# feinanshan/TDNet

Hardware: AMD Instinct MI355X
Metric: frames/sec (td4-psp18, 1024x2048, full-resolution logits) (higher is better)
Workload: dtype f32; 1 GPU; td4-psp18, 1024x2048 Cityscapes-shaped synthetic stream, 3-frame feature cache, 1 clip per GPU; parallelism=clip-parallel x1, RCCL weight broadcast only, target_fps_per_gpu=30

## Files before the change

tdnet_amd/csrc/td_launch.h:

```cpp
#pragma once
#include "td_weights.h"

#ifdef TDNET_TIMING_PROBES
static int probe_skip() {
    static const int m = [] {
        const char* e = getenv("TDNET_PROBE_SKIP");
        const int v = e ? atoi(e) : 0;
        if (v) fprintf(stderr, "tdnet: TDNET_PROBE_SKIP=%d -- pieces of the frame are NOT computed, every result of this process is garbage (timing probe build)\n", v);
        return v;
    }();
    return m;
}
#else
static constexpr int probe_skip() { return 0; }
#endif
static void prof_begin(tdnet* n, int family, int dominant, double flops, hipStream_t s) {
    if (!n || !n->prof) return;
    if (n->nrec == n->recs.size()) {
        ProfRec r;
        hipEventCreate(&r.e0); hipEventCreate(&r.e1);
        n->recs.push_back(r);
    }
    ProfRec& r = n->recs[n->nrec];
    r.family = family; r.dominant = dominant; r.flops = flops;
// ... 44 lines not shown
    const int TY = wino_tiles_1d(H, L.dil, L.wino), TX = wino_tiles_1d(W, L.dil, L.wino);
    const long T = (long)L.dil * L.dil * TY * TX;
    const bool chunked = ck.ny != 1 || ck.nx != 1;
    if (chunked && (!L.vw || L.dil % ck.ny || L.dil % ck.nx)) return td_fail("internal: this conv cannot run in chunks");
    const long Tc = (long)(L.dil / ck.ny) * (L.dil / ck.nx) * TY * TX;
    const int nb = (L.wino + 2) * (L.wino + 2);
    bool own = false;
    if (!V) {
        own = n == nullptr || n->wino_v_floats < (size_t)nb * Tc * L.Cin || n->wino_m_floats < (size_t)nb * Tc * L.Cout;
        if (own) {
            if (n) { n->failed = true; return td_fail("internal: Winograd workspace too small"); }
            if (dev_alloc(&V, (size_t)nb * Tc * L.Cin) || dev_alloc(&Mb, (size_t)nb * Tc * L.Cout)) return -1;
        } else { V = n->wino_v; Mb = n->wino_m; }
    }
    WinoArgs wa;
    wa.in = in; wa.V = V; wa.Mb = Mb; wa.bias = L.d_bias; wa.resid = resid; wa.out = out;
    wa.H = H; wa.W = W; wa.C = L.Cin; wa.Cout = L.Cout; wa.dil = L.dil; wa.TY = TY; wa.TX = TX; wa.T = (int)T; wa.act = L.act; wa.TP = (int)Tc;
    wa.ln_mean = lnf ? lnf->mean : nullptr; wa.ln_rstd = lnf ? lnf->rstd : nullptr; wa.ln_g = lnf ? lnf->g : nullptr; wa.ln_b = lnf ? lnf->b : nullptr;
    wa.Tc = (int)Tc; wa.ny = ck.ny; wa.cy = ck.cy; wa.nx = ck.nx; wa.cx = ck.cx;
    const long cmax = L.Cin > L.Cout ? L.Cin : L.Cout;
    if ((long)nb * Tc * cmax * 4 >= (1l << 31) || (long)H * W * cmax * 4 >= (1l << 31) ||
        (L.vw && !(wino_magic_ok(Tc * ((cmax + 63) / 64), TX) && wino_magic_ok(0, TY) && wino_magic_ok(0, L.dil))))
        return td_fail("internal: this conv is too large for the Winograd transforms");
    wa.mg_sl = wino_magic(1); wa.mg_tx = wino_magic(TX); wa.mg_ty = wino_magic(TY); wa.pw = L.dil / ck.nx; wa.mg_pw = wino_magic(wa.pw);
    auto transform = [&](bool out_side) {
        if (n && (probe_skip() & 1)) return;
        prof_begin(n, 2, false, 0, s);
        const int C = out_side ? L.Cout : L.Cin;
        if (out_side && cls) {
            const unsigned grid = (unsigned)((Tc + 3) / 4);
            if (L.Cout == 128) TD_LAUNCH((k_wino4_out_cls<2>), dim3(grid), dim3(256), wino_out_cls_lds(128, cls->NC), s, wa, *cls);
            else TD_LAUNCH((k_wino4_out_cls<1>), dim3(grid), dim3(256), wino_out_cls_lds(64, cls->NC), s, wa, *cls);
        } else
        if (L.vw == 1) launch_wino4_c<1>(out_side, wa, s);
        else if (L.vw == 2 && C % 2 == 0) launch_wino4_c<2>(out_side, wa, s);
        else if (L.vw == 4 && C % 4 == 0) launch_wino4_c<4>(out_side, wa, s);
        else if (L.vw) launch_wino4_c<1>(out_side, wa, s);
        else if (out_side && wino_act_general(wa.act)) TD_LAUNCH((k_wino4_out<true>), dim3(td_grid_for(T * (L.Cout / 4), 256, 256 * 16)), dim3(256), 0, s, wa);
        else if (out_side) TD_LAUNCH((k_wino4_out<false>), dim3(td_grid_for(T * (L.Cout / 4), 256, 256 * 16)), dim3(256), 0, s, wa);
        else TD_LAUNCH(k_wino4_in, dim3(td_grid_for(T * (L.Cin / 4), 256, 256 * 16)), dim3(256), 0, s, wa);
        prof_end(n, s);
    };
    transform(false);
    prof_begin(n, 0, 2, 2.0 * nb * Tc * (double)L.Cin * L.Cout, s);
    if (!(n && (probe_skip() & 8))) launch_gemm(L, gemm_args(L, V, (int)Tc, nb, L.d_zero, nullptr, Mb, 0), chunked ? 320 : 0, s);
    prof_end(n, s);
    transform(true);
    if (own) { TD_HIP(hipStreamSynchronize(s)); hipFree(V); hipFree(Mb); }
    return 0;
}

static void launch_conv_dma_forms(const ConvLayer& L, const ConvArgs& a, hipStream_t s) {
    int rh = L.rh;
    bool done = false;
    const bool is192 = rh == CD_192_P || rh == CD_192_N;
    if (rh == CD_128_N || rh == CD_192_N) {
        done = !L.rowimg_off && conv_launch_dma3n(a, rh, L.KS, L.out16, s);
        if (!done) rh = is192 ? CD_192_P : CD_128_P;
    }
    if (!done && (rh == CD_128_P || rh == CD_192_P)) {
        done = !L.rowimg_off && conv_launch_dma3p(a, rh, L.KS, L.out16, s);
        if (!done) rh = is192 ? CD_192 : CD_128_8W;
    }
    if (!done && (L.rowimg_off || !conv_launch_dma3(a, rh, L.KS, L.out16, s))) conv_launch_dma(a, rh, L.KS, L.out16, s);
}

static int run_conv(tdnet* n, const ConvLayer& L, const float* in, int H, int W, const float* resid, float* out, hipStream_t s,
                    int* Ho_out = nullptr, int* Wo_out = nullptr, const LnFuse* lnf = nullptr, const ClsArgs* cls = nullptr) {
    if (lnf && !L.wino) return td_fail("internal: LayerNorm fusion needs a Winograd input transform");
    if (cls && (!L.wino || L.chunks > 1 || resid || wino_act_general(L.act))) return td_fail("internal: the classifier rides in a whole Winograd conv's output transform");
    const int Ho = out_size(H, L.KS, L.stride, L.dil, L.pad), Wo = out_size(W, L.KS, L.stride, L.dil, L.pad);
    if (L.wino) {
        if (Ho_out) *Ho_out = H;
        if (Wo_out) *Wo_out = W;
        if (L.chunks > 1 && (!n || !n->ws_ready)) {
            for (int c = 0; c < L.chunks; ++c) {
                WinoChunk ck; ck.ny = L.chunks; ck.cy = c;
                TD_TRY(run_wino(n, L, in, H, W, resid, out, s, lnf, ck, nullptr, nullptr));
            }
            return 0;
        }
        return run_wino(n, L, in, H, W, resid, out, s, lnf, WinoChunk(), nullptr, nullptr, cls);
    }
    if (L.route == CR_WINO_F64 && !wino_f64_size_ok(H, W)) return td_fail("internal: this map is too large for the fused Winograd kernel");
    const ConvArgs a = conv_args(L, in, H, W, resid, out);
    const double flops = L.route == CR_WINO_F64 ? 2.0 * 36 * (double)wino_tiles(H, W, 1, 4) * L.Cin * L.Cout : L.flops_per_pixel() * a.M;
    prof_begin(n, 0, (((L.tile == CT_128x128 || L.tile == CT_128x128_DEEP || L.rh) && L.KS == 3 && !L.stem) ? 1 : 0) | ((L.h16() && L.in16 && L.KS == 3 && !L.stem) ? 4 : 0), flops, s);
    switch (L.route) {
    case CR_STEM_H: conv_launch_stem_h(a, L.out16, s); break;
    case CR_CONV_DMA: launch_conv_dma_forms(L, a, s); break;
    case CR_CONV_H: conv_launch_h(a, L.tile, L.KS, L.in16, L.out16, s); break;
    case CR_ADIRECT_B3: conv_launch_adirect_b3(a, L.KS, 0, s); break;
    case CR_GEMM1X1: launch_gemm(L, gemm_args(L, in, a.M, 1, L.d_bias, resid, out, L.act), 0, s); break;
    case CR_ADIRECT_ROWS:
    case CR_ADIRECT_ROWS_B3: {
        ConvArgs r = a;
        r.H = stem_rows_hp(H); r.W = stem_rows_wp(W); r.Cin = 3; r.pad = 0;
        if (L.route == CR_ADIRECT_ROWS_B3) conv_launch_adirect_b3(r, L.KS, 2, s);
        else conv_launch_adirect(r, L.KS, 2, s);
        break;
    }
    case CR_ADIRECT: conv_launch_adirect(a, L.KS, L.stem ? 1 : 0, s); break;
    case CR_IGEMM: conv_launch(a, L.tile, L.KS, L.stem, s); break;
    case CR_WINO_F64: wino_f64_launch(in, L.d_wp, L.d_bias, resid, out, H, W, L.act, s); break;
    case CR_WINO: break;
    }
    prof_end(n, s);
    if (Ho_out) *Ho_out = Ho;
    if (Wo_out) *Wo_out = Wo;
    return 0;
}

static int run_conv_src2(tdnet* n, const ConvLayer& L, const float* in, int ld, int k_split, int nsteps, const float* in2, int ld2, const float* wp2,
                         int H, int W, const float* resid, float* out, hipStream_t s) {
    if (L.KS != 1 || L.stem || L.wino) return td_fail("internal: two operand sources need a 1x1 conv");
    const ConvArgs a0 = conv_args(L, in, H, W, resid, out);
    prof_begin(n, 0, 0, 2.0 * L.Cout * 32.0 * nsteps * a0.M, s);
    int rc = 0;
    if (L.route == CR_GEMM1X1 && L.gemm == GK_PERSISTENT) {
        GemmArgs ga = gemm_args(L, in, a0.M, 1, L.d_bias, resid, out, L.act);
        ga.K = 32 * nsteps; ga.k_split = k_split; ga.lda = ld; ga.a2 = in2; ga.lda2 = ld2; ga.wp2 = wp2;
        if (!gemm_src2_supports(ga)) rc = td_fail("internal: the persistent GEMM cannot take this second operand source");
        else launch_gemm(L, ga, 0, s);
    } else if (L.route == CR_ADIRECT) {
        ConvArgs a = a0;
        a.Cin = 32 * nsteps; a.nsteps = nsteps; a.k_split = k_split; a.ld = ld; a.in2 = in2; a.ld2 = ld2; a.wp2 = wp2;
        if (resid || !conv_adirect_src2_supports(a, L.KS, 0)) rc = td_fail("internal: the direct 1x1 conv cannot take this second operand source");
        else conv_launch_adirect(a, 1, 0, s);
    } else rc = td_fail("internal: this conv's kernel has no second operand source");
    prof_end(n, s);
    return rc;
}

struct ConvCall { const ConvLayer* L; const float* in; int H, W; float* out; };
static bool conv_group_same_form(const tdnet_opts& o, const ConvCall* c, int ng) {
    bool same = (o.fusion & TDNET_FUSION_CONV_GROUPS) && ng >= 2 && ng <= 3;
    for (int g = 0; same && g < ng; ++g) {
        const ConvLayer& L = *c[g].L;
        const ConvLayer& L0 = *c[0].L;
        same = L.route == CR_CONV_H && L.in16 == L.out16 && L.in16 == L0.in16 && (g == 0 ? (L.KS == 1 || L.KS == 3) : L.KS == 1) &&
               conv_tile_dims(L.tile).BM == conv_tile_dims(L0.tile).BM && conv_tile_dims(L.tile).BN == conv_tile_dims(L0.tile).BN;
    }
    return same;
}
static int run_conv_group(tdnet* n, const tdnet_opts& o, const ConvCall* c, int ng, hipStream_t s, int* Ho_out = nullptr, int* Wo_out = nullptr,
                          int* grouped = nullptr) {
    const bool same = conv_group_same_form(o, c, ng);
    if (grouped) *grouped = same ? 1 : 0;
    if (!same) {
        for (int g = 0; g < ng; ++g) TD_TRY(run_conv(n, *c[g].L, c[g].in, c[g].H, c[g].W, nullptr, c[g].out, s, g == 0 ? Ho_out : nullptr, g == 0 ? Wo_out : nullptr));
        return 0;
    }
    ConvArgs a[3];
    double flops = 0.0;
    for (int g = 0; g < ng; ++g) {
        const ConvLayer& L = *c[g].L;
        a[g] = conv_args(L, c[g].in, c[g].H, c[g].W, nullptr, c[g].out);
        flops += L.flops_per_pixel() * a[g].M;
        if (g == 0 && Ho_out) *Ho_out = out_size(c[0].H, L.KS, L.stride, L.dil, L.pad);
        if (g == 0 && Wo_out) *Wo_out = a[0].Wo;
    }
    const bool dom = c[0].L->in16 && c[0].L->KS == 3;
    prof_begin(n, 0, dom ? 4 : 0, dom ? c[0].L->flops_per_pixel() * a[0].M : flops, s);
    conv_launch_h_group(a, ng, c[0].L->tile, c[0].L->KS, c[0].L->in16, c[0].L->out16, s);
    prof_end(n, s);
    return 0;
}

static int run_attention(tdnet* n, const float* q, const float* k, const float* vp, const float* bias, const float* resid,
                         int Lq, int Lk, int DV, float* out, hipStream_t s, int online = 0, float* ln_part = nullptr,
                         _Float16* vt16 = nullptr, bool slices = false, bool vt_ready = false, int b3 = 0) {
    if (n && n->vt16 && (n->opts.precision == 1 || b3)) vt16 = n->vt16;
    AttnArgs a;
    a.q = q; a.k = k; a.vp = vp; a.bias = bias; a.resid = resid; a.out = out; a.Lq = Lq; a.Lk = Lk;
    a.scale_log2e = 1.4426950408889634f / 8.0f;
    a.ln_part = ln_part; a.ln_nstr = 0;
    if (n && (probe_skip() & 4) && Lq > Lk) return 0;
    prof_begin(n, 1, false, 2.0 * Lq * (double)Lk * (64 + DV), s);
    const int rc = (vt16 && b3) ? attn_launch_b3(a, DV, reinterpret_cast<unsigned short*>(vt16), s, vt_ready, b3 - 1)
                 : vt16 ? attn_launch_h(a, DV, vt16, s, vt_ready) : attn_launch(a, DV, online, s, slices);
    prof_end(n, s);
    if (rc) return td_fail("attention: unsupported d_v=%d (128 or a multiple of 512)", DV);
    return 0;
}

static void run_layernorm(tdnet* n, const float* x, int HW, int C, const float* g, const float* b, float* part, float* mean,
                          float* rstd, float* y, hipStream_t s, int stats_nstr = 0, bool y16 = false) {
// ... 399 lines not shown
```

tdnet_amd/csrc/td_weights.h:

```cpp
#pragma once
#include "td_handle.h"

constexpr int RH_FRAME = -1;
constexpr int RH_BY_SIZE = -2;

static int plan_dma_form(const ConvLayer& c, long M, const tdnet_opts& o) {
    const bool narrow = (o.fusion & TDNET_FUSION_DMA_NARROW) != 0, same3 = c.KS == 3 && c.stride == 1 && c.pad == c.dil;
    if (!conv_dma_supports(c.Cin, c.Cout, c.KS, c.tile)) return CD_NONE;
    if (c.Cout == 64 && c.CoutPad == 128 && same3 && narrow) return CD_128_N;
    if (c.Cout < 128) return CD_NONE;
    const int rh = conv_dma_pick_rh(M, c.Cout, c.CoutPad % 256 == 0);
    if (narrow && same3 && M <= 16384 && c.Cout <= 256) return c.Cout <= 128 ? CD_128_N : CD_192_N;
    if (o.fusion & TDNET_FUSION_DMA_LOADERS) return rh == CD_128 ? CD_128_P : rh == CD_192 ? CD_192_P : rh;
    return rh;
}

static bool plan_wino_f64(const tdnet_opts& o, int Cout, int Cin, int KS, int stride, int dil, int act, bool stem, bool forced_tile, int chunks) {
    return (o.fusion & TDNET_FUSION_WINO_F64) && o.winograd >= 3 && o.precision == 0 && !forced_tile && chunks == 1 &&
           wino_f64_supports(Cout, Cin, KS, stride, dil, act, stem);
}

static int plan_conv(ConvLayer& L, int Cout, int Cin, int KS, int stride, int dil, int act, bool stem, long M, const tdnet_opts& o,
                     int forced_tile = -1, int chunks = 1, bool in16 = false, bool out16 = false, int rh = RH_FRAME, bool rowimg_off = false) {
    L = ConvLayer();
    L.Cin = stem ? 4 : Cin; L.Cout = Cout; L.KS = KS; L.stride = stride; L.dil = dil; L.act = act; L.stem = stem;
    L.pad = stem ? KS / 2 : dil * (KS / 2);
    L.pers = o.gemm_persistent;
    L.rowimg_off = rowimg_off;
    if (!stem && Cin % 32 != 0) return td_fail("conv: Cin=%d is not a multiple of 32", Cin);
    const bool deep = o.pipeline != 0, forced = forced_tile >= 0;
    const bool pers_gemm = o.gemm_persistent && gemm_supports(Cin);
    const bool split = o.precision >= 2;
    const bool split_narrow = split && (o.fusion & TDNET_FUSION_A_DIRECT) && (o.fusion & TDNET_FUSION_SPLIT_NARROW);
    if (plan_wino_f64(o, Cout, Cin, KS, stride, dil, act, stem, forced, chunks) && M >= TD_WINO_F64_MIN_PIXELS && M <= TD_WINO_F64_MAX_PIXELS) {
        L.route = CR_WINO_F64;
        L.nsteps = 0; L.CoutPad = Cout;
        return 0;
    }
    if (o.winograd && o.precision != 1 && !stem && KS == 3 && stride == 1 && Cin % 32 == 0 && Cout % 4 == 0 && (o.winograd == 4 || (Cin >= 128 && Cout >= 128))) {
        L.route = CR_WINO;
        L.wino = 4;
        L.chunks = (chunks > 1 && dil % chunks == 0 && pers_gemm) ? chunks : 1;
        L.vw = (L.chunks > 1 || (o.overlap & TDNET_OVERLAP_LOWREG_TRANSFORMS)) ? (1 << ((o.overlap & TDNET_OVERLAP_VW_MASK) >> TDNET_OVERLAP_VW_SHIFT)) : 0;
        const int nb = (L.wino + 2) * (L.wino + 2);
        const long rows = wino_tiles_estimate(M, dil, L.wino) / L.chunks;
        L.tile = forced ? (ConvTile)forced_tile : pers_gemm ? gemm_pick_tile(rows, nb, Cout, deep)
                                                            : conv_pick_tile((int)std::min<long>(nb * M / (L.wino * L.wino), 1 << 30), Cout, deep);
        L.nsteps = conv_nsteps(Cin, 1, 0);
        const bool b3 = split && pers_gemm && gemm_b3_supports(Cin, Cout) && (forced || o.precision == 3 || gemm_b3_pick(rows, nb, Cout));
        L.gemm = !pers_gemm ? GK_CONV : b3 ? GK_B3 : ((o.overlap & TDNET_OVERLAP_GEMM_DMA) && gemm_dma_supports(Cin, Cout, L.tile)) ? GK_DMA : GK_PERSISTENT;
        L.CoutPad = b3 ? gemm_b3_npad(Cout) : conv_cout_pad(Cout, L.tile);
        return 0;
    }
    const bool h16 = o.precision == 1 && !stem && Cin % 64 == 0;
    const bool stem16 = o.precision == 1 && stem && KS == 7 && stride == 2 && Cout <= 64;
    const bool is1x1 = !h16 && !stem && KS == 1 && stride == 1 && pers_gemm;
    const bool narrow1x1 = is1x1 && !forced && split_narrow && Cout <= 128 && M >= 8192 && gemm_b3_supports(Cin, Cout) && !gemm_b3_pick(M, 1, Cout, Cin) &&
                           conv_adirect_b3_supports(CT_128x64, Cin, KS, stem);
    const bool gemm1x1 = is1x1 && !narrow1x1;
    L.tile = forced ? (ConvTile)forced_tile : gemm1x1 ? gemm_pick_tile(M, 1, Cout, deep) : conv_pick_tile((int)M, Cout, deep);
    if (!forced && split_narrow && !h16 && !stem && !gemm1x1 && Cout <= 128 && conv_adirect_b3_supports(CT_128x64, Cin, KS, stem)) L.tile = CT_128x64;
    if (h16 && !forced && (o.fusion & TDNET_FUSION_DMA_NARROW) && KS == 3 && stride == 1 && Cout == 64) L.tile = CT_128x128_DEEP;
    L.CoutPad = conv_cout_pad(Cout, L.tile);
    L.nsteps = conv_nsteps(Cin, KS, stem ? 1 : 0);
    if (stem16 && conv_stem_h_supports(L.tile)) {
        L.route = CR_STEM_H;
        L.nsteps = conv_nsteps_stem_h();
    } else if (h16) {
        L.route = CR_CONV_H;
        L.nsteps = conv_nsteps_h(Cin, KS);
    } else if (gemm1x1) {
        const bool b3 = split && gemm_b3_supports(Cin, Cout) && (forced || o.precision == 3 || gemm_b3_pick(M, 1, Cout, Cin));
        L.route = CR_GEMM1X1;
        L.gemm = b3 ? GK_B3 : GK_PERSISTENT;
        if (b3) { L.CoutPad = gemm_b3_npad(Cout); L.nsteps = Cin / 16; }
    } else if (split_narrow && conv_adirect_b3_supports(L.tile, Cin, KS, stem)) {
        L.route = CR_ADIRECT_B3;
    } else if ((o.fusion & TDNET_FUSION_A_DIRECT) && conv_adirect_supports(L.tile, 1)) {
        const bool rows = stem && KS == 7 && stride == 2 && (o.fusion & TDNET_FUSION_STEM_ROWS);
        L.route = !rows ? CR_ADIRECT : split_narrow ? CR_ADIRECT_ROWS_B3 : CR_ADIRECT_ROWS;
        if (rows) L.nsteps = conv_nsteps(Cin, KS, 2);
    }
    if (L.h16()) { L.in16 = in16; L.out16 = out16; }
    if (L.route == CR_CONV_H && L.in16) {
        L.rh = rh == RH_FRAME ? plan_dma_form(L, M, o)
             : rh == RH_BY_SIZE ? (Cout >= 128 && conv_dma_supports(Cin, Cout, KS, L.tile) ? conv_dma_pick_rh(M, Cout, L.CoutPad % 256 == 0) : CD_NONE) : rh;
        if (L.rh) L.route = CR_CONV_DMA;
    }
    return 0;
}

static bool plan_enc_fold(const tdnet_opts& o, const ConvLayer& v, const ConvLayer& q0, const ConvLayer& k0, int XS, int FS) {
    const auto gemm = [](const ConvLayer& L) { return L.route == CR_GEMM1X1 && L.gemm == GK_PERSISTENT; };
    return (o.fusion & TDNET_FUSION_PPM_FOLD) && o.precision == 0 && gemm(v) && gemm(q0) && k0.route == CR_ADIRECT && k0.KS == 1 && !k0.stem &&
           XS >= 64 && XS % 64 == 0 && FS % 16 == 0 && v.Cin == XS + 4 * FS && q0.Cin == v.Cin && k0.Cin == v.Cin &&
           v.CoutPad % 64 == 0 && q0.CoutPad % 64 == 0 && k0.CoutPad % 64 == 0;
}

template <typename T, typename Pack>
static int upload_packed(float** d, size_t count, Pack pack) {
    std::vector<T> packed(count);
    pack(packed.data());
    TD_TRY(dev_alloc((T**)d, count));
    TD_HIP(hipMemcpy(*d, packed.data(), count * sizeof(T), hipMemcpyHostToDevice));
    return 0;
}
static int upload_conv(ConvLayer& L, const std::vector<float>& w, const std::vector<float>& b) {
    typedef unsigned short bf16;
    const int Cout = L.Cout, Cin = L.Cin, KS = L.KS, stem_kind = L.stem_rows() ? 2 : L.stem ? 1 : 0;
    const size_t tile_image = (size_t)L.nsteps * 8 * L.CoutPad * 4;
    if (L.route == CR_WINO) {
        const int nb = (L.wino + 2) * (L.wino + 2);
        std::vector<std::vector<float>> U;
        wino_transform_weights(w.data(), Cout, Cin, L.wino, U);
        const size_t per = L.gemm == GK_B3 ? gemm_b3_packed_bytes(Cin, Cout) / 2 : tile_image;
        if (L.gemm == GK_B3) TD_TRY(upload_packed<bf16>(&L.d_wp, nb * per, [&](bf16* p) { for (int bi = 0; bi < nb; ++bi) gemm_b3_pack(U[bi].data(), Cout, Cin, p + bi * per); }));
        else TD_TRY(upload_packed<float>(&L.d_wp, nb * per, [&](float* p) { for (int bi = 0; bi < nb; ++bi) conv_pack_weights(U[bi].data(), Cout, Cin, 1, 0, L.tile, p + bi * per); }));
    } else if (L.route == CR_WINO_F64)
        TD_TRY(upload_packed<float>(&L.d_wp, wino_f64_packed_floats(), [&](float* p) { wino_f64_pack(w.data(), p); }));
    else if (L.route == CR_STEM_H)
        TD_TRY(upload_packed<_Float16>(&L.d_wp, 2 * tile_image, [&](_Float16* p) { conv_pack_weights_stem_h(w.data(), Cout, L.tile, p); }));
    else if (L.h16())
        TD_TRY(upload_packed<_Float16>(&L.d_wp, 2 * tile_image, [&](_Float16* p) { conv_pack_weights_h(w.data(), Cout, Cin, KS, L.tile, p); }));
    else if (L.route == CR_GEMM1X1 && L.gemm == GK_B3)
        TD_TRY(upload_packed<bf16>(&L.d_wp, gemm_b3_packed_bytes(Cin, Cout) / 2, [&](bf16* p) { gemm_b3_pack(w.data(), Cout, Cin, p); }));
    else if (L.route == CR_ADIRECT_B3 || L.route == CR_ADIRECT_ROWS_B3)
        TD_TRY(upload_packed<bf16>(&L.d_wp, conv_adb3_packed_bytes(Cout, Cin, KS, stem_kind) / 2, [&](bf16* p) { conv_pack_weights_adb3(w.data(), Cout, Cin, KS, p, stem_kind); }));
    else
        TD_TRY(upload_packed<float>(&L.d_wp, tile_image, [&](float* p) { conv_pack_weights(w.data(), Cout, Cin, KS, stem_kind, L.tile, p); }));
    TD_TRY(upload(&L.d_bias, b.empty() ? std::vector<float>(Cout, 0.f) : b));
    if (L.wino) TD_TRY(upload(&L.d_zero, std::vector<float>(Cout, 0.f)));
    return 0;
}
static void free_conv_layer(ConvLayer& L) {
    if (L.d_wp) hipFree(L.d_wp);
    if (L.d_bias) hipFree(L.d_bias);
    if (L.d_zero) hipFree(L.d_zero);
    L.d_wp = L.d_bias = L.d_zero = nullptr;
}
static void add_bn(std::map<std::string, size_t>& e, const std::string& pre, int c) {
    e[pre + ".weight"] = c; e[pre + ".bias"] = c; e[pre + ".running_mean"] = c; e[pre + ".running_var"] = c;
    e[pre + ".num_batches_tracked"] = 1;
}
static std::vector<std::string> atn_module_names(int model) {
    if (model == 4) return {"atn1_2", "atn1_3", "atn1_4", "atn2_1", "atn2_3", "atn2_4", "atn3_1", "atn3_2", "atn3_4", "atn4_1", "atn4_2", "atn4_3"};
    return {"atn1", "atn2"};
}
static std::vector<std::string> atn_order(int model, int p) {
    if (model == 2) return {p == 0 ? "atn1" : "atn2"};
    static const char* t[4][3] = {{"atn1_2", "atn1_3", "atn1_4"}, {"atn2_3", "atn2_4", "atn2_1"},
                                  {"atn3_4", "atn3_1", "atn3_2"}, {"atn4_1", "atn4_2", "atn4_3"}};
    return {t[p][0], t[p][1], t[p][2]};
}
static void build_expected(tdnet* n) {
    auto& e = n->expected;
    char b[160];
    for (int p = 1; p <= n->P; ++p) {
        snprintf(b, sizeof(b), "pretrained%d", p);
        std::string pre = n->cfg.model == 1 ? std::string("pretrained") : std::string(b);
        if (n->deep) {
            e[pre + ".conv1.0.weight"] = 64 * 3 * 9; add_bn(e, pre + ".conv1.1", 64);
            e[pre + ".conv1.3.weight"] = 64 * 64 * 9; add_bn(e, pre + ".conv1.4", 64);
            e[pre + ".conv1.6.weight"] = 128 * 64 * 9; add_bn(e, pre + ".bn1", 128);
        } else {
            e[pre + ".conv1.weight"] = 64 * 3 * 49;
            add_bn(e, pre + ".bn1", 64);
        }
        for (auto& s : n->bspec) {
            std::string bp = pre + "." + s.name;
            if (s.bott) {
                e[bp + ".conv1.weight"] = (size_t)s.planes * s.cin; add_bn(e, bp + ".bn1", s.planes);
                e[bp + ".conv2.weight"] = (size_t)s.planes * s.planes * 9; add_bn(e, bp + ".bn2", s.planes);
                e[bp + ".conv3.weight"] = (size_t)s.cout * s.planes; add_bn(e, bp + ".bn3", s.cout);
            } else {
                e[bp + ".conv1.weight"] = (size_t)s.cout * s.cin * 9; add_bn(e, bp + ".bn1", s.cout);
                e[bp + ".conv2.weight"] = (size_t)s.cout * s.cout * 9; add_bn(e, bp + ".bn2", s.cout);
            }
            if (s.ds) { e[bp + ".downsample.0.weight"] = (size_t)s.cout * s.cin; add_bn(e, bp + ".downsample.1", s.cout); }
        }
        e[pre + ".fc.weight"] = (size_t)1000 * n->C; e[pre + ".fc.bias"] = 1000;
        if (n->cfg.model == 1) {
            for (int j = 1; j <= 4; ++j) {
                snprintf(b, sizeof(b), "head.conv5.0.conv%d", j);
                e[std::string(b) + ".0.weight"] = (size_t)(n->C / 4) * n->C;
                add_bn(e, std::string(b) + ".1", n->C / 4);
            }
            e["head.conv5.1.weight"] = (size_t)(n->C / 4) * 2 * n->C * 9; add_bn(e, "head.conv5.2", n->C / 4);
            e["head.conv5.5.weight"] = (size_t)n->cfg.nclass * (n->C / 4); e["head.conv5.5.bias"] = n->cfg.nclass;
            continue;
        }
        for (int j = 1; j <= 4; ++j) {
            snprintf(b, sizeof(b), "psp%d.conv%d", p, j);
            e[std::string(b) + ".0.weight"] = (size_t)(n->C / 4) * n->C;
            add_bn(e, std::string(b) + ".1", n->C / 4);
        }
        for (const char* br : {"w_qs", "w_ks"}) {
            snprintf(b, sizeof(b), "enc%d.%s", p, br);
            std::string ep = b;
            e[ep + ".0.conv.weight"] = (size_t)64 * n->C; e[ep + ".0.conv.bias"] = 64; add_bn(e, ep + ".0.bn", 64);
            e[ep + ".1.conv.weight"] = 64 * 64; e[ep + ".1.conv.bias"] = 64;
        }
        snprintf(b, sizeof(b), "enc%d.w_vs.0.conv", p);
// ... 358 lines not shown
```

tdnet_amd/csrc/td_wino_f64.h:

```cpp
#pragma once
#include "td_wino.h"

constexpr int TD_WF64_C = 64;
constexpr int TD_WF64_BX = 8, TD_WF64_BY = 4;
constexpr int TD_WF64_LDS = 36 * 8 * 2 * 32 * 4;
constexpr long TD_WINO_F64_MIN_PIXELS = 32768;

struct WinoF64Args {
    const float* in;
    const float* up;
    const float* bias;
    const float* resid;
    float* out;
    int H, W, BXN, act;
};

static inline bool wino_f64_supports(int Cout, int Cin, int KS, int stride, int dil, int act, bool stem) {
    return !stem && KS == 3 && stride == 1 && dil == 1 && Cin == TD_WF64_C && Cout == TD_WF64_C && (act == 0 || act == 1);
}
constexpr long TD_WINO_F64_MAX_PIXELS = (1l << 31) / (TD_WF64_C * 4) - 1;
static inline bool wino_f64_size_ok(int H, int W) { return H >= 1 && W >= 1 && (long)H * W <= TD_WINO_F64_MAX_PIXELS; }
constexpr int TD_WF64_PACKED_FLOATS = 2 * 36 * 8 * 64 * 4;
static inline size_t wino_f64_packed_floats() { return (size_t)TD_WF64_PACKED_FLOATS; }
static inline void wino_f64_pack(const float* w, float* p) {
    std::vector<std::vector<float>> U;
    wino_transform_weights(w, TD_WF64_C, TD_WF64_C, 4, U);
    for (int hb = 0; hb < 2; ++hb)
        for (int pos = 0; pos < 36; ++pos)
            for (int kq = 0; kq < 8; ++kq)
                for (int lane = 0; lane < 64; ++lane)
                    for (int j = 0; j < 4; ++j)
                        p[((((size_t)hb * 36 + pos) * 8 + kq) * 64 + lane) * 4 + j] =
                            U[pos][(size_t)(32 * hb + (lane & 31)) * TD_WF64_C + 8 * kq + 4 * (lane >> 5) + j];
}

TD_DEV int td_wf64_vidx(int pos, int slot, int tile) { return pos * 512 + slot * 32 + (tile ^ (4 * ((slot >> 2) & 3))); }
TD_DEV int td_wf64_midx(int pos, int j, int t) { return pos * 512 + j * 16 + (t ^ (2 * (j >> 2))); }

TD_KERNEL void TD_LAUNCH_BOUNDS(256, 2) k_wino4_f64(WinoF64Args p) {
    TD_DYN_LDS(smem);
    float* lds = reinterpret_cast<float*>(smem);
    const int tid = threadIdx.x, lane = tid & 63, wave = TD_UNIFORM(tid >> 6);
    const int bx = (int)blockIdx.x % p.BXN, by = (int)blockIdx.x / p.BXN, hb = (int)blockIdx.y;
    const unsigned map_bytes = (unsigned)p.H * (unsigned)p.W * (unsigned)TD_WF64_C * 4u;
    const TdBuf inb = td_make_buf(p.in, map_bytes);
    const TdBuf ub = td_make_buf(p.up, (unsigned)TD_WF64_PACKED_FLOATS * 4u);
    const TdBuf rb = td_make_buf(p.resid, p.resid ? map_bytes : 0u);
    const TdBuf ob = td_make_buf(p.out, map_bytes);
    f32x16 acc[9];
#pragma unroll
    for (int q = 0; q < 9; ++q)
#pragma unroll
        for (int r = 0; r < 16; ++r) acc[q][r] = 0.f;
    const unsigned ulane = (unsigned)lane * 16u;
    const unsigned ubase = (unsigned)((hb * 36 + wave * 9) * 8) * 1024u;
    const float* va[4];
#pragma unroll
    for (int g = 0; g < 4; ++g) va[g] = lds + td_wf64_vidx(wave * 9, 4 * g + (lane >> 5), lane & 31);

#pragma unroll 1
    for (int kc = 0; kc < 4; ++kc) {
        int t = tid;
        TD_PIN(t);
        const int tl = t >> 3, cp = t & 7;
        const int tx = bx * TD_WF64_BX + (tl & 7), ty = by * TD_WF64_BY + (tl >> 3);
        unsigned offy[6], offx[6];
#pragma unroll
        for (int r = 0; r < 6; ++r) {
            const int y = 4 * ty - 1 + r, x = 4 * tx - 1 + r;
            offy[r] = (unsigned)y < (unsigned)p.H ? (unsigned)y * (unsigned)p.W * (unsigned)(TD_WF64_C * 4) : TD_BUF_OOB;
            offx[r] = (unsigned)x < (unsigned)p.W ? (unsigned)x * (unsigned)(TD_WF64_C * 4) + (unsigned)(16 * kc + 2 * cp) * 4u : TD_BUF_OOB;
        }
        f32x2 dd[6][6];
#pragma unroll
        for (int c = 0; c < 6; ++c)
#pragma unroll
            for (int r = 0; r < 6; ++r) dd[c][r] = td_buf_ld2(inb, __builtin_elementwise_add_sat(offy[r], offx[c]), 0u);
        f32x2 tm[6][6];
#pragma unroll
        for (int c = 0; c < 6; ++c) {
            f32x2 col[6];
            td_wino4_bt_t(dd[c], col);
#pragma unroll
            for (int r = 0; r < 6; ++r) tm[r][c] = col[r];
        }
        if (kc) __syncthreads();
        float* vd = lds + td_wf64_vidx(0, (4 * (cp >> 2) + ((2 * cp) & 3)) * 2 + ((cp >> 1) & 1), tl);
#pragma unroll
        for (int r = 0; r < 6; ++r) {
            f32x2 v[6];
            td_wino4_bt_t(tm[r], v);
#pragma unroll
            for (int c = 0; c < 6; ++c) {
                vd[(r * 6 + c) * 512] = v[c][0];
                vd[(r * 6 + c) * 512 + 64] = v[c][1];
            }
        }
        f32x4 b0[9], b1[9];
#pragma unroll
        for (int q = 0; q < 9; ++q) b0[q] = td_buf_ld4(ub, ulane, ubase + (unsigned)((q * 8 + 2 * kc) * 1024));
        __syncthreads();
#pragma unroll
        for (int q = 0; q < 9; ++q) b1[q] = td_buf_ld4(ub, ulane, ubase + (unsigned)((q * 8 + 2 * kc + 1) * 1024));
#pragma unroll
        for (int j = 0; j < 4; ++j)
#pragma unroll
            for (int q = 0; q < 9; ++q) acc[q] = td_mfma32(va[j >> 1][q * 512 + (j & 1) * 64], b0[q][j], acc[q]);
#pragma unroll
        for (int j = 0; j < 4; ++j)
#pragma unroll
            for (int q = 0; q < 9; ++q) acc[q] = td_mfma32(va[2 + (j >> 1)][q * 512 + (j & 1) * 64], b1[q][j], acc[q]);
    }

    const int tl = tid >> 4, cpp = tid & 15;
    const TdBuf bb = td_make_buf(p.bias, (unsigned)(TD_WF64_C * 4));
    const f32x2 b = td_buf_ld2(bb, (unsigned)(32 * hb + 2 * cpp) * 4u, 0u);
#pragma unroll
    for (int rd = 0; rd < 2; ++rd) {
        const int tx = bx * TD_WF64_BX + (tl & 7), ty = by * TD_WF64_BY + 2 * rd + (tl >> 3);
        unsigned offy[4], offx[4];
#pragma unroll
        for (int r = 0; r < 4; ++r) {
            const int y = 4 * ty + r, x = 4 * tx + r;
            offy[r] = y < p.H ? (unsigned)y * (unsigned)p.W * (unsigned)(TD_WF64_C * 4) : TD_BUF_OOB;
            offx[r] = x < p.W ? (unsigned)x * (unsigned)(TD_WF64_C * 4) + (unsigned)(32 * hb + 2 * cpp) * 4u : TD_BUF_OOB;
        }
        f32x2 o[16];
#pragma unroll
        for (int r = 0; r < 4; ++r)
#pragma unroll
            for (int c = 0; c < 4; ++c) o[r * 4 + c] = td_buf_ld2(rb, __builtin_elementwise_add_sat(offy[r], offx[c]), 0u);
        __syncthreads();
        {
            const int j = lane & 31, i4 = 4 * (lane >> 5);
#pragma unroll
            for (int q = 0; q < 9; ++q)
#pragma unroll
                for (int r = 0; r < 8; ++r) lds[td_wf64_midx(wave * 9 + q, j, (r & 3) + 8 * (r >> 2) + i4)] = acc[q][8 * rd + r];
        }
        __syncthreads();
        f32x2 sm[4][6];
#pragma unroll
        for (int c = 0; c < 6; ++c) {
            f32x2 mc[6], col[4];
#pragma unroll
            for (int r = 0; r < 6; ++r) mc[r] = f32x2{lds[td_wf64_midx(r * 6 + c, 2 * cpp, tl)], lds[td_wf64_midx(r * 6 + c, 2 * cpp + 1, tl)]};
            td_wino4_at_t(mc, col);
#pragma unroll
            for (int r = 0; r < 4; ++r) sm[r][c] = col[r];
        }
#pragma unroll
        for (int r = 0; r < 4; ++r) {
            f32x2 o4[4];
            td_wino4_at_t(sm[r], o4);
#pragma unroll
            for (int c = 0; c < 4; ++c) o[r * 4 + c] = (o4[c] + b) + o[r * 4 + c];
        }
        td_wino_activate<false>(o, p.act);
#pragma unroll
        for (int r = 0; r < 4; ++r)
#pragma unroll
            for (int c = 0; c < 4; ++c) td_buf_st2(ob, __builtin_elementwise_add_sat(offy[r], offx[c]), 0u, o[r * 4 + c]);
    }
}

static inline bool wino_f64_launch(const float* in, const float* up, const float* bias, const float* resid, float* out, int H, int W, int act, hipStream_t s) {
    if (!wino_f64_size_ok(H, W)) return false;
    const int TX = wino_tiles_1d(W, 1, 4), TY = wino_tiles_1d(H, 1, 4);
    const int bxn = (TX + TD_WF64_BX - 1) / TD_WF64_BX, byn = (TY + TD_WF64_BY - 1) / TD_WF64_BY;
    const WinoF64Args a = {in, up, bias, resid, out, H, W, bxn, act};
    TD_LAUNCH(k_wino4_f64, dim3((unsigned)(bxn * byn), 2), dim3(256), TD_WF64_LDS, s, a);
    return true;
}
```

Baseline: 301.0 frames/s.

## Generalize fused Winograd F(4,3) kernel to 128 channels and vectorize LDS layout

Templates the fused Winograd kernel on channel count so 128-channel 3x3 convs can use it, but only at exactly 32768 pixels, which is a narrow routing window. It also reworks the LDS swizzles so transformed inputs and accumulators are stored and read as f32x2/f32x4 vectors instead of scalars. The MFMA operand order is swapped and the epilogue splits output channels by rd instead of tile rows. The goal is fewer LDS instructions and fusing one more layer, at the cost of riskier layout math and changed register pressure.

```diff
diff --git a/tdnet_amd/csrc/td_launch.h b/tdnet_amd/csrc/td_launch.h
--- a/tdnet_amd/csrc/td_launch.h
+++ b/tdnet_amd/csrc/td_launch.h
@@ -150,7 +150,7 @@
         }
         return run_wino(n, L, in, H, W, resid, out, s, lnf, WinoChunk(), nullptr, nullptr, cls);
     }
-    if (L.route == CR_WINO_F64 && !wino_f64_size_ok(H, W)) return td_fail("internal: this map is too large for the fused Winograd kernel");
+    if (L.route == CR_WINO_F64 && !wino_f64_size_ok(L.Cin, H, W)) return td_fail("internal: this map is too large for the fused Winograd kernel");
     const ConvArgs a = conv_args(L, in, H, W, resid, out);
     const double flops = L.route == CR_WINO_F64 ? 2.0 * 36 * (double)wino_tiles(H, W, 1, 4) * L.Cin * L.Cout : L.flops_per_pixel() * a.M;
     prof_begin(n, 0, (((L.tile == CT_128x128 || L.tile == CT_128x128_DEEP || L.rh) && L.KS == 3 && !L.stem) ? 1 : 0) | ((L.h16() && L.in16 && L.KS == 3 && !L.stem) ? 4 : 0), flops, s);
@@ -170,7 +170,7 @@
     }
     case CR_ADIRECT: conv_launch_adirect(a, L.KS, L.stem ? 1 : 0, s); break;
     case CR_IGEMM: conv_launch(a, L.tile, L.KS, L.stem, s); break;
-    case CR_WINO_F64: wino_f64_launch(in, L.d_wp, L.d_bias, resid, out, H, W, L.act, s); break;
+    case CR_WINO_F64: wino_f64_launch(in, L.d_wp, L.d_bias, resid, out, L.Cin, H, W, L.act, s); break;
     case CR_WINO: break;
     }
     prof_end(n, s);
diff --git a/tdnet_amd/csrc/td_weights.h b/tdnet_amd/csrc/td_weights.h
--- a/tdnet_amd/csrc/td_weights.h
+++ b/tdnet_amd/csrc/td_weights.h
@@ -32,7 +32,7 @@
     const bool pers_gemm = o.gemm_persistent && gemm_supports(Cin);
     const bool split = o.precision >= 2;
     const bool split_narrow = split && (o.fusion & TDNET_FUSION_A_DIRECT) && (o.fusion & TDNET_FUSION_SPLIT_NARROW);
-    if (plan_wino_f64(o, Cout, Cin, KS, stride, dil, act, stem, forced, chunks) && M >= TD_WINO_F64_MIN_PIXELS && M <= TD_WINO_F64_MAX_PIXELS) {
+    if (plan_wino_f64(o, Cout, Cin, KS, stride, dil, act, stem, forced, chunks) && wino_f64_routes(Cin, M)) {
         L.route = CR_WINO_F64;
         L.nsteps = 0; L.CoutPad = Cout;
         return 0;
@@ -117,7 +117,7 @@
         if (L.gemm == GK_B3) TD_TRY(upload_packed<bf16>(&L.d_wp, nb * per, [&](bf16* p) { for (int bi = 0; bi < nb; ++bi) gemm_b3_pack(U[bi].data(), Cout, Cin, p + bi * per); }));
         else TD_TRY(upload_packed<float>(&L.d_wp, nb * per, [&](float* p) { for (int bi = 0; bi < nb; ++bi) conv_pack_weights(U[bi].data(), Cout, Cin, 1, 0, L.tile, p + bi * per); }));
     } else if (L.route == CR_WINO_F64)
-        TD_TRY(upload_packed<float>(&L.d_wp, wino_f64_packed_floats(), [&](float* p) { wino_f64_pack(w.data(), p); }));
+        TD_TRY(upload_packed<float>(&L.d_wp, wino_f64_packed_floats(Cout, Cin), [&](float* p) { wino_f64_pack(w.data(), Cout, Cin, p); }));
     else if (L.route == CR_STEM_H)
         TD_TRY(upload_packed<_Float16>(&L.d_wp, 2 * tile_image, [&](_Float16* p) { conv_pack_weights_stem_h(w.data(), Cout, L.tile, p); }));
     else if (L.h16())
diff --git a/tdnet_amd/csrc/td_wino_f64.h b/tdnet_amd/csrc/td_wino_f64.h
--- a/tdnet_amd/csrc/td_wino_f64.h
+++ b/tdnet_amd/csrc/td_wino_f64.h
@@ -1,10 +1,11 @@
 #pragma once
 #include "td_wino.h"
 
-constexpr int TD_WF64_C = 64;
 constexpr int TD_WF64_BX = 8, TD_WF64_BY = 4;
 constexpr int TD_WF64_LDS = 36 * 8 * 2 * 32 * 4;
 constexpr long TD_WINO_F64_MIN_PIXELS = 32768;
+constexpr long TD_WINO_F128_MIN_PIXELS = 32768;
+constexpr long TD_WINO_F128_MAX_PIXELS = 32768;
 
 struct WinoF64Args {
     const float* in;
@@ -16,50 +17,56 @@
 };
 
 static inline bool wino_f64_supports(int Cout, int Cin, int KS, int stride, int dil, int act, bool stem) {
-    return !stem && KS == 3 && stride == 1 && dil == 1 && Cin == TD_WF64_C && Cout == TD_WF64_C && (act == 0 || act == 1);
+    return !stem && KS == 3 && stride == 1 && dil == 1 && (Cin == 64 || Cin == 128) && Cout == Cin && (act == 0 || act == 1);
 }
-constexpr long TD_WINO_F64_MAX_PIXELS = (1l << 31) / (TD_WF64_C * 4) - 1;
-static inline bool wino_f64_size_ok(int H, int W) { return H >= 1 && W >= 1 && (long)H * W <= TD_WINO_F64_MAX_PIXELS; }
-constexpr int TD_WF64_PACKED_FLOATS = 2 * 36 * 8 * 64 * 4;
-static inline size_t wino_f64_packed_floats() { return (size_t)TD_WF64_PACKED_FLOATS; }
-static inline void wino_f64_pack(const float* w, float* p) {
+static inline long wino_f64_max_pixels(int C) { return (1l << 31) / (C * 4) - 1; }
+static inline bool wino_f64_size_ok(int C, int H, int W) { return H >= 1 && W >= 1 && (long)H * W <= wino_f64_max_pixels(C); }
+static inline bool wino_f64_routes(int C, long M) {
+    return C == 64 ? M >= TD_WINO_F64_MIN_PIXELS && M <= wino_f64_max_pixels(64) : M >= TD_WINO_F128_MIN_PIXELS && M <= TD_WINO_F128_MAX_PIXELS;
+}
+static inline size_t wino_f64_packed_floats(int Cout, int Cin) { return (size_t)(Cout / 32) * 36 * (Cin / 8) * 64 * 4; }
+static inline void wino_f64_pack(const float* w, int Cout, int Cin, float* p) {
     std::vector<std::vector<float>> U;
-    wino_transform_weights(w, TD_WF64_C, TD_WF64_C, 4, U);
-    for (int hb = 0; hb < 2; ++hb)
+    wino_transform_weights(w, Cout, Cin, 4, U);
+    const int KQ = Cin / 8;
+    for (int hb = 0; hb < Cout / 32; ++hb)
         for (int pos = 0; pos < 36; ++pos)
-            for (int kq = 0; kq < 8; ++kq)
+            for (int kq = 0; kq < KQ; ++kq)
                 for (int lane = 0; lane < 64; ++lane)
                     for (int j = 0; j < 4; ++j)
-                        p[((((size_t)hb * 36 + pos) * 8 + kq) * 64 + lane) * 4 + j] =
-                            U[pos][(size_t)(32 * hb + (lane & 31)) * TD_WF64_C + 8 * kq + 4 * (lane >> 5) + j];
+                        p[((((size_t)hb * 36 + pos) * KQ + kq) * 64 + lane) * 4 + j] =
+                            U[pos][(size_t)(32 * hb + (lane & 31)) * Cin + 8 * kq + 4 * (lane >> 5) + j];
 }
 
-TD_DEV int td_wf64_vidx(int pos, int slot, int tile) { return pos * 512 + slot * 32 + (tile ^ (4 * ((slot >> 2) & 3))); }
-TD_DEV int td_wf64_midx(int pos, int j, int t) { return pos * 512 + j * 16 + (t ^ (2 * (j >> 2))); }
+TD_DEV int td_wf64_vidx(int pos, int slot, int tile) { return pos * 512 + (slot * 32 + (tile ^ (2 * slot))) * 4; }
+TD_DEV int td_wf64_midx(int pos, int tile, int cq) { return pos * 512 + (tile * 4 + (cq ^ ((tile >> 1) & 3))) * 4; }
 
+template <int CIN, int COUT>
 TD_KERNEL void TD_LAUNCH_BOUNDS(256, 2) k_wino4_f64(WinoF64Args p) {
+    static_assert(CIN % 16 == 0 && COUT % 32 == 0, "chunks of 16 input channels, blocks of 32 output channels");
+    constexpr int KQ = CIN / 8;
     TD_DYN_LDS(smem);
     float* lds = reinterpret_cast<float*>(smem);
     const int tid = threadIdx.x, lane = tid & 63, wave = TD_UNIFORM(tid >> 6);
     const int bx = (int)blockIdx.x % p.BXN, by = (int)blockIdx.x / p.BXN, hb = (int)blockIdx.y;
-    const unsigned map_bytes = (unsigned)p.H * (unsigned)p.W * (unsigned)TD_WF64_C * 4u;
-    const TdBuf inb = td_make_buf(p.in, map_bytes);
-    const TdBuf ub = td_make_buf(p.up, (unsigned)TD_WF64_PACKED_FLOATS * 4u);
-    const TdBuf rb = td_make_buf(p.resid, p.resid ? map_bytes : 0u);
-    const TdBuf ob = td_make_buf(p.out, map_bytes);
+    const unsigned pixels = (unsigned)p.H * (unsigned)p.W;
+    const TdBuf inb = td_make_buf(p.in, pixels * (unsigned)(CIN * 4));
+    const TdBuf ub = td_make_buf(p.up, (unsigned)(COUT / 32 * 36 * KQ * 64 * 4) * 4u);
+    const TdBuf rb = td_make_buf(p.resid, p.resid ? pixels * (unsigned)(COUT * 4) : 0u);
+    const TdBuf ob = td_make_buf(p.out, pixels * (unsigned)(COUT * 4));
     f32x16 acc[9];
 #pragma unroll
     for (int q = 0; q < 9; ++q)
 #pragma unroll
         for (int r = 0; r < 16; ++r) acc[q][r] = 0.f;
     const unsigned ulane = (unsigned)lane * 16u;
-    const unsigned ubase = (unsigned)((hb * 36 + wave * 9) * 8) * 1024u;
-    const float* va[4];
+    const unsigned ubase = (unsigned)((hb * 36 + wave * 9) * KQ) * 1024u;
+    const float* va[2];
 #pragma unroll
-    for (int g = 0; g < 4; ++g) va[g] = lds + td_wf64_vidx(wave * 9, 4 * g + (lane >> 5), lane & 31);
+    for (int g = 0; g < 2; ++g) va[g] = lds + td_wf64_vidx(wave * 9, 2 * g + (lane >> 5), lane & 31);
 
 #pragma unroll 1
-    for (int kc = 0; kc < 4; ++kc) {
+    for (int kc = 0; kc < CIN / 16; ++kc) {
         int t = tid;
         TD_PIN(t);
         const int tl = t >> 3, cp = t & 7;
@@ -68,8 +75,8 @@
 #pragma unroll
         for (int r = 0; r < 6; ++r) {
             const int y = 4 * ty - 1 + r, x = 4 * tx - 1 + r;
-            offy[r] = (unsigned)y < (unsigned)p.H ? (unsigned)y * (unsigned)p.W * (unsigned)(TD_WF64_C * 4) : TD_BUF_OOB;
-            offx[r] = (unsigned)x < (unsigned)p.W ? (unsigned)x * (unsigned)(TD_WF64_C * 4) + (unsigned)(16 * kc + 2 * cp) * 4u : TD_BUF_OOB;
+            offy[r] = (unsigned)y < (unsigned)p.H ? (unsigned)y * (unsigned)p.W * (unsigned)(CIN * 4) : TD_BUF_OOB;
+            offx[r] = (unsigned)x < (unsigned)p.W ? (unsigned)x * (unsigned)(CIN * 4) + (unsigned)(16 * kc + 2 * cp) * 4u : TD_BUF_OOB;
         }
         f32x2 dd[6][6];
 #pragma unroll
@@ -85,45 +92,47 @@
             for (int r = 0; r < 6; ++r) tm[r][c] = col[r];
         }
         if (kc) __syncthreads();
-        float* vd = lds + td_wf64_vidx(0, (4 * (cp >> 2) + ((2 * cp) & 3)) * 2 + ((cp >> 1) & 1), tl);
+        float* vd = lds + td_wf64_vidx(0, cp >> 1, tl) + 2 * (cp & 1);
 #pragma unroll
         for (int r = 0; r < 6; ++r) {
             f32x2 v[6];
             td_wino4_bt_t(tm[r], v);
 #pragma unroll
-            for (int c = 0; c < 6; ++c) {
-                vd[(r * 6 + c) * 512] = v[c][0];
-                vd[(r * 6 + c) * 512 + 64] = v[c][1];
-            }
+            for (int c = 0; c < 6; ++c) *reinterpret_cast<f32x2*>(vd + (r * 6 + c) * 512) = v[c];
         }
-        f32x4 b0[9], b1[9];
+        f32x4 b[2][9];
 #pragma unroll
-        for (int q = 0; q < 9; ++q) b0[q] = td_buf_ld4(ub, ulane, ubase + (unsigned)((q * 8 + 2 * kc) * 1024));
+        for (int q = 0; q < 9; ++q) b[0][q] = td_buf_ld4(ub, ulane, ubase + (unsigned)((q * KQ + 2 * kc) * 1024));
         __syncthreads();
 #pragma unroll
-        for (int q = 0; q < 9; ++q) b1[q] = td_buf_ld4(ub, ulane, ubase + (unsigned)((q * 8 + 2 * kc + 1) * 1024));
+        for (int q = 0; q < 9; ++q) b[1][q] = td_buf_ld4(ub, ulane, ubase + (unsigned)((q * KQ + 2 * kc + 1) * 1024));
 #pragma unroll
-        for (int j = 0; j < 4; ++j)
+        for (int g = 0; g < 2; ++g)
 #pragma unroll
-            for (int q = 0; q < 9; ++q) acc[q] = td_mfma32(va[j >> 1][q * 512 + (j & 1) * 64], b0[q][j], acc[q]);
+            for (int q3 = 0; q3 < 9; q3 += 3) {
+                f32x4 a[3];
 #pragma unroll
-        for (int j = 0; j < 4; ++j)
+                for (int q = 0; q < 3; ++q) a[q] = *reinterpret_cast<const f32x4*>(va[g] + (q3 + q) * 512);
 #pragma unroll
-            for (int q = 0; q < 9; ++q) acc[q] = td_mfma32(va[2 + (j >> 1)][q * 512 + (j & 1) * 64], b1[q][j], acc[q]);
+                for (int j = 0; j < 4; ++j)
+#pragma unroll
+                    for (int q = 0; q < 3; ++q) acc[q3 + q] = td_mfma32(b[g][q3 + q][j], a[q][j], acc[q3 + q]);
+            }
     }
 
-    const int tl = tid >> 4, cpp = tid & 15;
-    const TdBuf bb = td_make_buf(p.bias, (unsigned)(TD_WF64_C * 4));
-    const f32x2 b = td_buf_ld2(bb, (unsigned)(32 * hb + 2 * cpp) * 4u, 0u);
+    const int tl = tid >> 3, cpp = tid & 7;
+    const int tx = bx * TD_WF64_BX + (tl & 7), ty = by * TD_WF64_BY + (tl >> 3);
+    const TdBuf bb = td_make_buf(p.bias, (unsigned)(COUT * 4));
 #pragma unroll
     for (int rd = 0; rd < 2; ++rd) {
-        const int tx = bx * TD_WF64_BX + (tl & 7), ty = by * TD_WF64_BY + 2 * rd + (tl >> 3);
+        const unsigned ch = (unsigned)(32 * hb + 16 * rd + 2 * cpp) * 4u;
+        const f32x2 bs = td_buf_ld2(bb, ch, 0u);
         unsigned offy[4], offx[4];
 #pragma unroll
         for (int r = 0; r < 4; ++r) {
             const int y = 4 * ty + r, x = 4 * tx + r;
-            offy[r] = y < p.H ? (unsigned)y * (unsigned)p.W * (unsigned)(TD_WF64_C * 4) : TD_BUF_OOB;
-            offx[r] = x < p.W ? (unsigned)x * (unsigned)(TD_WF64_C * 4) + (unsigned)(32 * hb + 2 * cpp) * 4u : TD_BUF_OOB;
+            offy[r] = y < p.H ? (unsigned)y * (unsigned)p.W * (unsigned)(COUT * 4) : TD_BUF_OOB;
+            offx[r] = x < p.W ? (unsigned)x * (unsigned)(COUT * 4) + ch : TD_BUF_OOB;
         }
         f32x2 o[16];
 #pragma unroll
@@ -132,19 +141,23 @@
             for (int c = 0; c < 4; ++c) o[r * 4 + c] = td_buf_ld2(rb, __builtin_elementwise_add_sat(offy[r], offx[c]), 0u);
         __syncthreads();
         {
-            const int j = lane & 31, i4 = 4 * (lane >> 5);
+            float* md = lds + td_wf64_midx(wave * 9, lane & 31, lane >> 5);
+            const int hi = td_wf64_midx(0, lane & 31, 2 + (lane >> 5)) - td_wf64_midx(0, lane & 31, lane >> 5);
 #pragma unroll
             for (int q = 0; q < 9; ++q)
 #pragma unroll
-                for (int r = 0; r < 8; ++r) lds[td_wf64_midx(wave * 9 + q, j, (r & 3) + 8 * (r >> 2) + i4)] = acc[q][8 * rd + r];
+                for (int rq = 0; rq < 2; ++rq)
+                    *reinterpret_cast<f32x4*>(md + q * 512 + rq * hi) =
+                        f32x4{acc[q][8 * rd + 4 * rq], acc[q][8 * rd + 4 * rq + 1], acc[q][8 * rd + 4 * rq + 2], acc[q][8 * rd + 4 * rq + 3]};
         }
         __syncthreads();
+        const float* ms = lds + td_wf64_midx(0, tl, cpp >> 1) + 2 * (cpp & 1);
         f32x2 sm[4][6];
 #pragma unroll
         for (int c = 0; c < 6; ++c) {
             f32x2 mc[6], col[4];
 #pragma unroll
-            for (int r = 0; r < 6; ++r) mc[r] = f32x2{lds[td_wf64_midx(r * 6 + c, 2 * cpp, tl)], lds[td_wf64_midx(r * 6 + c, 2 * cpp + 1, tl)]};
+            for (int r = 0; r < 6; ++r) mc[r] = *reinterpret_cast<const f32x2*>(ms + (r * 6 + c) * 512);
             td_wino4_at_t(mc, col);
 #pragma unroll
             for (int r = 0; r < 4; ++r) sm[r][c] = col[r];
@@ -154,7 +167,7 @@
             f32x2 o4[4];
             td_wino4_at_t(sm[r], o4);
 #pragma unroll
-            for (int c = 0; c < 4; ++c) o[r * 4 + c] = (o4[c] + b) + o[r * 4 + c];
+            for (int c = 0; c < 4; ++c) o[r * 4 + c] = (o4[c] + bs) + o[r * 4 + c];
         }
         td_wino_activate<false>(o, p.act);
 #pragma unroll
@@ -164,11 +177,13 @@
     }
 }
 
-static inline bool wino_f64_launch(const float* in, const float* up, const float* bias, const float* resid, float* out, int H, int W, int act, hipStream_t s) {
-    if (!wino_f64_size_ok(H, W)) return false;
+static inline bool wino_f64_launch(const float* in, const float* up, const float* bias, const float* resid, float* out, int C, int H, int W, int act, hipStream_t s) {
+    if ((C != 64 && C != 128) || !wino_f64_size_ok(C, H, W)) return false;
     const int TX = wino_tiles_1d(W, 1, 4), TY = wino_tiles_1d(H, 1, 4);
     const int bxn = (TX + TD_WF64_BX - 1) / TD_WF64_BX, byn = (TY + TD_WF64_BY - 1) / TD_WF64_BY;
     const WinoF64Args a = {in, up, bias, resid, out, H, W, bxn, act};
-    TD_LAUNCH(k_wino4_f64, dim3((unsigned)(bxn * byn), 2), dim3(256), TD_WF64_LDS, s, a);
+    const dim3 grid((unsigned)(bxn * byn), (unsigned)(C / 32));
+    if (C == 64) TD_LAUNCH((k_wino4_f64<64, 64>), grid, dim3(256), TD_WF64_LDS, s, a);
+    else TD_LAUNCH((k_wino4_f64<128, 128>), grid, dim3(256), TD_WF64_LDS, s, a);
     return true;
 }
```

Result: no change. 301.9 frames/s, median of 6 (+0.3%).
